# gabrielfnayres/new-vit

Hardware: AMD Instinct MI355X
Metric: volumes_per_sec_mst_dinov2_fwd (higher is better)
Workload: dtype bf16; 1 GPU; MST-DINOv2 (DinoV2ClassifierSlice, ViT-S/14) forward, 4 volumes/GPU of 64x512x512 bf16 zero-padded to 518x518 (N=1370 tokens/slice); global_batch_volumes=4, slices=64, parallelism=single GPU, weights=synthetic (mst.synth seed 2), random init of the reference architecture

## Files before the change

### new-vit_amd/build.py

```python
#!/usr/bin/env python3
from __future__ import annotations

import argparse
import os
import shutil
import subprocess
import sys
from concurrent.futures import ThreadPoolExecutor
from pathlib import Path

HERE = Path(__file__).resolve().parent
CSRC = HERE / "csrc"
OBJ = HERE / "build"
LIB = Path(os.environ.get("MST_BUILD_LIB", HERE / "mst" / "hip" / "libmst_hip.so"))
FLAGS = ["--offload-arch=gfx950", "-O3", "-std=c++17", "-fPIC", "-Wall", "-Wno-unused-function",
         "-Wno-unused-variable", "-Wno-unused-but-set-variable"]
PER_FILE_FLAGS = {"k_block16s.hip": ["-fno-slp-vectorize"],
                  "k_attn16.hip": ["-mllvm", "-amdgpu-mfma-vgpr-form"], "k_attn32.hip": ["-mllvm", "-amdgpu-mfma-vgpr-form"],
                  "k_attn16_train.hip": ["-mllvm", "-amdgpu-mfma-vgpr-form"]}


def hipcc() -> str:
    for c in (os.environ.get("HIPCC"), shutil.which("hipcc"), "/opt/rocm/bin/hipcc"):
        if c and Path(c).exists():
            return c
    raise RuntimeError("hipcc not found (ROCm toolchain required to build libmst_hip.so)")


def newer(src: Path, dst: Path, deps) -> bool:
    if not dst.exists():
        return True
    t = dst.stat().st_mtime
    return any(p.stat().st_mtime > t for p in [src, *deps])


def build(force: bool = False, jobs: int = 8, verbose: bool = True) -> Path:
    global OBJ
    cc = hipcc()
    extra = os.environ.get("MST_EXTRA_FLAGS", "").split()
    if extra:
        OBJ = HERE / ("build_" + "_".join(f.strip("-").replace("=", "") for f in extra))
        FLAGS.extend(f for f in extra if f not in FLAGS)
    OBJ.mkdir(exist_ok=True)
    headers = list(CSRC.glob("*.h")) + [HERE.parent / "include" / "mst_hip.h", Path(__file__)]
    srcs = sorted(CSRC.glob("*.hip"))
    todo = [s for s in srcs if force or newer(s, OBJ / (s.stem + ".o"), headers)]

    def compile_one(src: Path):
        cmd = [cc, *FLAGS, *PER_FILE_FLAGS.get(src.name, []), "-c", str(src), "-o", str(OBJ / (src.stem + ".o"))]
        r = subprocess.run(cmd, capture_output=True, text=True)
        return src, r

    with ThreadPoolExecutor(max_workers=max(1, jobs)) as ex:
        for src, r in ex.map(compile_one, todo):
            if verbose and (r.stderr.strip() or r.returncode):
                sys.stderr.write(r.stderr)
            if r.returncode:
                raise RuntimeError(f"hipcc failed on {src.name}")
            if verbose:
                print(f"[build] {src.name}")
    objs = [OBJ / (s.stem + ".o") for s in srcs]
    if force or todo or not LIB.exists():
        cmd = [cc, "--offload-arch=gfx950", "-shared", "-fPIC", "-o", str(LIB), *map(str, objs)]
        r = subprocess.run(cmd, capture_output=True, text=True)
        if r.returncode:
            sys.stderr.write(r.stderr)
            raise RuntimeError("link failed")
        if verbose:
            print(f"[build] linked {LIB}")
    return LIB


if __name__ == "__main__":
    ap = argparse.ArgumentParser()
    ap.add_argument("--force", action="store_true")
    ap.add_argument("--jobs", type=int, default=8)
    a = ap.parse_args()
    build(a.force, a.jobs)
```

### new-vit_amd/csrc/k_gemm16_wreg.hip

```cpp
#include <cstdlib>

#include "mst_common.h"

namespace {

constexpr int KD = GEMM16_WREG_TILE.bk, BN = GEMM16_WREG_TILE.bn, CH = GEMM16_WREG_TILE.bm;
constexpr int ROWB = KD * 2;
constexpr int SLOT = CH * ROWB;
constexpr int WREG_NSLOT = 4;
constexpr int NSLOT = WREG_NSLOT;
constexpr int STG_PITCH = ROWB + 16;
constexpr int STG_BYTES = CH * STG_PITCH;
constexpr int STG_OFF = NSLOT * SLOT;
constexpr int LDS_BYTES = STG_OFF + 2 * STG_BYTES;
constexpr int NKT = KD / 32;
constexpr int PPW = SLOT / 1024 / 8;
static_assert(NSLOT == 4, "the counted vmcnt table below is written for three chunks in flight");

#define WREG_RD(dst, base, imm) asm volatile("ds_read_b128 %0, %1 offset:%2" : "=v"(dst) : "v"(base), "n"(imm) : "memory")

template <typename T, bool BLK>
__global__ __launch_bounds__(512) __attribute__((amdgpu_waves_per_eu(2, 2))) void gemm16_wreg_kernel(
    const T* __restrict__ A, int64_t lda, const T* __restrict__ W, int64_t ldw, const float* __restrict__ bias, T* __restrict__ C,
    int64_t ldc, int M, int N, float col_scale, int scale_cols, int nchunks) {
    typedef typename V8<T>::type vec8;
    typedef __attribute__((ext_vector_type(4))) T out4;
    extern __shared__ __attribute__((aligned(16))) char smem[];
    const int lane = threadIdx.x & 63;
    const int wave = __builtin_amdgcn_readfirstlane(threadIdx.x >> 6);
    const int frow = lane & 15, kq = lane >> 4;

    const int xcd = blockIdx.x & 7, g = blockIdx.x >> 3, G = gridDim.x >> 3;
    const int tiles_n = N / BN;
    const int nt = g % tiles_n, jcu = g / tiles_n;
    const int c_nt = (G - nt + tiles_n - 1) / tiles_n;
    const int per_xcd = (nchunks + 7) >> 3;
    const int lo = xcd * per_xcd;
    const int hi = lo + per_xcd < nchunks ? lo + per_xcd : nchunks;
    const int n0 = nt * BN + wave * 48;
    const float cs = nt * BN < scale_cols ? col_scale : 1.f;

    vec8 w[3][NKT];
#pragma unroll
    for (int t = 0; t < 3; ++t) {
        const T* wr = W + (int64_t)(n0 + 12 * (frow >> 2) + 4 * t + (frow & 3)) * ldw + kq * 8;
#pragma unroll
        for (int kt = 0; kt < NKT; ++kt) w[t][kt] = *reinterpret_cast<const vec8*>(wr + kt * 32);
    }
    f32x4 b[3];
#pragma unroll
    for (int t = 0; t < 3; ++t) {
        b[t] = (f32x4){0.f, 0.f, 0.f, 0.f};
        if (bias) b[t] = *reinterpret_cast<const f32x4*>(bias + n0 + 12 * kq + 4 * t);
    }
#pragma unroll
    for (int t = 0; t < 3; ++t) {
        asm volatile("" : "+v"(b[t]));
#pragma unroll
        for (int kt = 0; kt < NKT; ++kt) asm volatile("" : "+v"(w[t][kt]));
    }

    unsigned dma_off[PPW];
#pragma unroll
    for (int u = 0; u < PPW; ++u) {
        const int o = (wave * PPW + u) * 1024 + lane * 16;
        const int r = o / ROWB;
        dma_off[u] = BLK ? (unsigned)o : (unsigned)(r * (int)lda * 2 + ((((o % ROWB) >> 4) ^ (r & 15)) << 4));
    }
    const int64_t chunk_bytes = BLK ? (int64_t)SLOT : (int64_t)CH * lda * 2;
    auto issue_piece = [&](int chunk, int slot, int u) {
        const char* base = reinterpret_cast<const char*>(A) + (int64_t)chunk * chunk_bytes;
        unsigned off = dma_off[u];
        const int valid = M - chunk * CH;
        if (!BLK && valid < CH) {
            const int o = (wave * PPW + u) * 1024 + lane * 16;
            int r = o / ROWB;
            const int ck = ((o % ROWB) >> 4) ^ (r & 15);
            r = r < valid ? r : valid - 1;
            off = (unsigned)(r * (int)lda * 2 + ck * 16);
        }
        __builtin_amdgcn_global_load_lds(GLB_PTR(base + off), LDS_PTR(smem + slot * SLOT + (wave * PPW + u) * 1024), 16, 0, 0);
    };

    int rb[4];
#pragma unroll
    for (int j = 0; j < 4; ++j) rb[j] = BLK ? (kq >> 1) * 1024 + (frow + 32 * (kq & 1)) * 16 : frow * ROWB + (((4 * j + kq) ^ frow) << 4);
    const int put_off = frow * STG_PITCH + wave * 96 + kq * 24;
    int fl_lds[3];
    unsigned fl_glb[3];
    int fl_row[3];
#pragma unroll
    for (int j = 0; j < 3; ++j) {
        const int q = lane + 64 * j;
        fl_row[j] = wave * 4 + q / 48;
        fl_lds[j] = fl_row[j] * STG_PITCH + (q % 48) * 16;
        fl_glb[j] = (unsigned)(fl_row[j] * (int)ldc * 2 + nt * BN * 2 + (q % 48) * 16);
    }
    f32x4 acc[2][3];
    auto put = [&](int it) {
        char* stg = smem + STG_OFF + (it & 1) * STG_BYTES + put_off;
#pragma unroll
        for (int mt = 0; mt < 2; ++mt)
#pragma unroll
            for (int t = 0; t < 3; ++t) {
                out4 pk;
#pragma unroll
                for (int i = 0; i < 4; ++i) pk[i] = (T)(acc[mt][t][i] * cs);
                *reinterpret_cast<out4*>(stg + mt * 16 * STG_PITCH + t * 8) = pk;
            }
    };
    auto flush_piece = [&](int chunk, int it, int j) {
        const char* stg = smem + STG_OFF + (it & 1) * STG_BYTES;
        char* cb = reinterpret_cast<char*>(C) + (int64_t)chunk * CH * ldc * 2;
        const int valid = M - chunk * CH;
        const u32x4 v = *reinterpret_cast<const u32x4*>(stg + fl_lds[j]);
        if (valid >= CH || fl_row[j] < valid) {
            __builtin_nontemporal_store(v, reinterpret_cast<u32x4*>(cb + fl_glb[j]));
        }
    };
    auto flush = [&](int chunk, int it) {
#pragma unroll
        for (int j = 0; j < 3; ++j) flush_piece(chunk, it, j);
    };

    int c = lo + jcu;
    if (c >= hi) return;
#pragma unroll
    for (int d = 0; d < NSLOT - 1; ++d)
        if (c + d * c_nt < hi) {
#pragma unroll
            for (int u = 0; u < PPW; ++u) issue_piece(c + d * c_nt, d, u);
        }

    int prev = -1, last_it = 0;
    for (int it = 0; c < hi; c += c_nt, ++it) {
        if (c + 2 * c_nt < hi) {
            if (it <= 1) asm volatile("s_waitcnt vmcnt(6)" ::: "memory");
            else if (it == 2) asm volatile("s_waitcnt vmcnt(9)" ::: "memory");
            else asm volatile("s_waitcnt vmcnt(12)" ::: "memory");
        } else {
            asm volatile("s_waitcnt vmcnt(0)" ::: "memory");
        }
        asm volatile("s_waitcnt lgkmcnt(0)\n\ts_barrier" ::: "memory");
        if (prev >= 0) flush(prev, it - 1);

        const int slot = it % NSLOT;
        const int nxt = c + (NSLOT - 1) * c_nt, nslot = (it + NSLOT - 1) % NSLOT;
        const bool more = nxt < hi;
        int rbs[4];
#pragma unroll
        for (int j = 0; j < 4; ++j) rbs[j] = rb[j] + slot * SLOT;
#pragma unroll
        for (int mt = 0; mt < 2; ++mt)
#pragma unroll
            for (int t = 0; t < 3; ++t) acc[mt][t] = b[t];

        u32x4 a[2][2];
        WREG_RD(a[0][0], rbs[0], 0);
        if constexpr (BLK) WREG_RD(a[0][1], rbs[0], 256);
        else WREG_RD(a[0][1], rbs[0], 16 * ROWB);
#pragma unroll
        for (int kt = 0; kt < NKT; ++kt) {
            const int cur = kt & 1;
            if (kt + 1 < NKT) {
                switch (kt + 1) {
#define WREG_NEXT(KN)                                                                  \
    case KN:                                                                           \
        if constexpr (BLK) {                                                           \
            WREG_RD(a[(KN) & 1][0], rbs[0], (KN) * 2048);                              \
            WREG_RD(a[(KN) & 1][1], rbs[0], (KN) * 2048 + 256);                        \
        } else {                                                                       \
            WREG_RD(a[(KN) & 1][0], rbs[(KN) & 3], ((KN) >> 2) * 256);                 \
            WREG_RD(a[(KN) & 1][1], rbs[(KN) & 3], 16 * ROWB + ((KN) >> 2) * 256);     \
        }                                                                              \
        break;
                    WREG_NEXT(1) WREG_NEXT(2) WREG_NEXT(3) WREG_NEXT(4) WREG_NEXT(5) WREG_NEXT(6)
                    WREG_NEXT(7) WREG_NEXT(8) WREG_NEXT(9) WREG_NEXT(10) WREG_NEXT(11)
#undef WREG_NEXT
                }
                asm volatile("s_waitcnt lgkmcnt(2)" : "+v"(a[cur][0]), "+v"(a[cur][1])::"memory");
            } else {
                asm volatile("s_waitcnt lgkmcnt(0)" : "+v"(a[cur][0]), "+v"(a[cur][1])::"memory");
            }
            const vec8 a0 = __builtin_bit_cast(vec8, a[cur][0]), a1 = __builtin_bit_cast(vec8, a[cur][1]);
#pragma unroll
            for (int t = 0; t < 3; ++t) {
                acc[0][t] = mfma16(w[t][kt], a0, acc[0][t]);
                acc[1][t] = mfma16(w[t][kt], a1, acc[1][t]);
            }
            if ((kt & 3) == 1) {
                __builtin_amdgcn_sched_barrier(0);
                if (more) issue_piece(nxt, nslot, kt >> 2);
                __builtin_amdgcn_sched_barrier(0);
            }
        }
        put(it);
        prev = c;
        last_it = it;
    }
    asm volatile("s_waitcnt lgkmcnt(0)\n\ts_barrier" ::: "memory");
    flush(prev, last_it);
}

template <typename T, bool BLK>
int launch_t(const gemm_args& g) {
    static mst_lds_once lds_once;
    auto kern = gemm16_wreg_kernel<T, BLK>;
    mst_allow_lds((const void*)kern, LDS_BYTES, &lds_once);
    const int nchunks = (int)((g.M + CH - 1) / CH);
    kern<<<dim3(mst_persistent_grid()), dim3(512), LDS_BYTES, g.s>>>((const T*)g.A, g.lda, (const T*)g.W, g.ldw, g.bias, (T*)g.C, g.ldc, (int)g.M,
                                                                      g.N, g.col_scale, g.scale_cols, nchunks);
    return mst_check_launch("gemm16_wreg");
}

}

int launch_gemm16_wreg(const gemm_args& g, int a_blocked) {
    if (a_blocked) {
        if (g.dt == MST_BF16) return launch_t<bf16_t, true>(g);
        if (g.dt == MST_F16) return launch_t<f16_t, true>(g);
    }
    if (g.dt == MST_BF16) return launch_t<bf16_t, false>(g);
    if (g.dt == MST_F16) return launch_t<f16_t, false>(g);
    mst_set_error("gemm16_wreg: bad operand dtype %d", g.dt);
    return MST_EINVAL;
}
```

Measured before the change: 166.3 volumes/s.

## Overlap wreg GEMM output flush with MFMA loop and specialize scaling epilogue

The output-tile flush is split into LDS reads, issued alongside the first A-fragment reads, and buffer stores issued after the first MFMA group. This hides the epilogue store latency behind compute instead of running it serially after the barrier. Row masking now relies on a buffer resource with a bounded extent rather than per-lane branches. The chunk loop is also instantiated separately for scaled and unscaled columns so the multiply is skipped when not needed, with packed conversion (and fma_mix for f16) and -fno-slp-vectorize added for this file. The cost is more live VGPRs for the staged flush data and code duplication from the two loop instantiations.

```diff
diff --git a/new-vit_amd/build.py b/new-vit_amd/build.py
--- a/new-vit_amd/build.py
+++ b/new-vit_amd/build.py
@@ -16,6 +16,7 @@
 FLAGS = ["--offload-arch=gfx950", "-O3", "-std=c++17", "-fPIC", "-Wall", "-Wno-unused-function",
          "-Wno-unused-variable", "-Wno-unused-but-set-variable"]
 PER_FILE_FLAGS = {"k_block16s.hip": ["-fno-slp-vectorize"],
+                  "k_gemm16_wreg.hip": ["-fno-slp-vectorize"],
                   "k_attn16.hip": ["-mllvm", "-amdgpu-mfma-vgpr-form"], "k_attn32.hip": ["-mllvm", "-amdgpu-mfma-vgpr-form"],
                   "k_attn16_train.hip": ["-mllvm", "-amdgpu-mfma-vgpr-form"]}
 
diff --git a/new-vit_amd/csrc/k_gemm16_wreg.hip b/new-vit_amd/csrc/k_gemm16_wreg.hip
--- a/new-vit_amd/csrc/k_gemm16_wreg.hip
+++ b/new-vit_amd/csrc/k_gemm16_wreg.hip
@@ -1,4 +1,5 @@
 #include <cstdlib>
+#include <type_traits>
 
 #include "mst_common.h"
 
@@ -24,7 +25,8 @@
     const T* __restrict__ A, int64_t lda, const T* __restrict__ W, int64_t ldw, const float* __restrict__ bias, T* __restrict__ C,
     int64_t ldc, int M, int N, float col_scale, int scale_cols, int nchunks) {
     typedef typename V8<T>::type vec8;
-    typedef __attribute__((ext_vector_type(4))) T out4;
+    typedef __attribute__((ext_vector_type(2))) T out2;
+    typedef __attribute__((ext_vector_type(2))) float f32x2;
     extern __shared__ __attribute__((aligned(16))) char smem[];
     const int lane = threadIdx.x & 63;
     const int wave = __builtin_amdgcn_readfirstlane(threadIdx.x >> 6);
@@ -38,7 +40,7 @@
     const int lo = xcd * per_xcd;
     const int hi = lo + per_xcd < nchunks ? lo + per_xcd : nchunks;
     const int n0 = nt * BN + wave * 48;
-    const float cs = nt * BN < scale_cols ? col_scale : 1.f;
+    const bool scaled = nt * BN < scale_cols && col_scale != 1.f;
 
     vec8 w[3][NKT];
 #pragma unroll
@@ -88,39 +90,52 @@
     const int put_off = frow * STG_PITCH + wave * 96 + kq * 24;
     int fl_lds[3];
     unsigned fl_glb[3];
-    int fl_row[3];
 #pragma unroll
     for (int j = 0; j < 3; ++j) {
         const int q = lane + 64 * j;
-        fl_row[j] = wave * 4 + q / 48;
-        fl_lds[j] = fl_row[j] * STG_PITCH + (q % 48) * 16;
-        fl_glb[j] = (unsigned)(fl_row[j] * (int)ldc * 2 + nt * BN * 2 + (q % 48) * 16);
+        const int row = wave * 4 + q / 48;
+        fl_lds[j] = row * STG_PITCH + (q % 48) * 16;
+        fl_glb[j] = (unsigned)(row * (int)ldc * 2 + nt * BN * 2 + (q % 48) * 16);
     }
     f32x4 acc[2][3];
-    auto put = [&](int it) {
+    auto put = [&](int it, auto sc_tag) {
+        constexpr bool SC = decltype(sc_tag)::value;
         char* stg = smem + STG_OFF + (it & 1) * STG_BYTES + put_off;
 #pragma unroll
         for (int mt = 0; mt < 2; ++mt)
 #pragma unroll
             for (int t = 0; t < 3; ++t) {
-                out4 pk;
-#pragma unroll
-                for (int i = 0; i < 4; ++i) pk[i] = (T)(acc[mt][t][i] * cs);
-                *reinterpret_cast<out4*>(stg + mt * 16 * STG_PITCH + t * 8) = pk;
+                f32x4 v = acc[mt][t];
+                u32x2 pk;
+                if constexpr (SC && std::is_same<T, f16_t>::value) {
+                    const float m1 = v[1] * col_scale, m2 = v[2] * col_scale;
+                    pk[0] = __builtin_bit_cast(unsigned, __builtin_convertvector((f32x2){m1, m1}, out2));
+                    pk[1] = __builtin_bit_cast(unsigned, __builtin_convertvector((f32x2){m2, m2}, out2));
+                    asm("v_fma_mixlo_f16 %0, %1, %2, 0" : "+v"(pk[0]) : "v"(col_scale), "v"(v[0]));
+                    asm("v_fma_mixhi_f16 %0, %1, %2, 0" : "+v"(pk[1]) : "v"(col_scale), "v"(v[3]));
+                } else {
+                    if constexpr (SC) {
+#pragma unroll
+                        for (int i = 0; i < 4; ++i) v[i] *= col_scale;
+                    }
+                    pk[0] = __builtin_bit_cast(unsigned, __builtin_convertvector((f32x2){v[0], v[1]}, out2));
+                    pk[1] = __builtin_bit_cast(unsigned, __builtin_convertvector((f32x2){v[2], v[3]}, out2));
+                }
+                *reinterpret_cast<u32x2*>(stg + mt * 16 * STG_PITCH + t * 8) = pk;
             }
     };
-    auto flush_piece = [&](int chunk, int it, int j) {
-        const char* stg = smem + STG_OFF + (it & 1) * STG_BYTES;
-        char* cb = reinterpret_cast<char*>(C) + (int64_t)chunk * CH * ldc * 2;
+    u32x4 fl[3] = {};
+    auto flush_reads = [&](int it) {
+        const int tile = STG_OFF + (it & 1) * STG_BYTES;
+#pragma unroll
+        for (int j = 0; j < 3; ++j) WREG_RD(fl[j], fl_lds[j] + tile, 0);
+    };
+    auto flush_stores = [&](int chunk) {
         const int valid = M - chunk * CH;
-        const u32x4 v = *reinterpret_cast<const u32x4*>(stg + fl_lds[j]);
-        if (valid >= CH || fl_row[j] < valid) {
-            __builtin_nontemporal_store(v, reinterpret_cast<u32x4*>(cb + fl_glb[j]));
-        }
-    };
-    auto flush = [&](int chunk, int it) {
-#pragma unroll
-        for (int j = 0; j < 3; ++j) flush_piece(chunk, it, j);
+        const __amdgpu_buffer_rsrc_t rows = __builtin_amdgcn_make_buffer_rsrc(
+            reinterpret_cast<char*>(C) + (int64_t)chunk * CH * ldc * 2, 0, (valid < CH ? valid : CH) * (int)ldc * 2, 0x00020000);
+#pragma unroll
+        for (int j = 0; j < 3; ++j) __builtin_amdgcn_raw_buffer_store_b128(fl[j], rows, (int)fl_glb[j], 0, 2);
     };
 
     int c = lo + jcu;
@@ -133,37 +148,38 @@
         }
 
     int prev = -1, last_it = 0;
-    for (int it = 0; c < hi; c += c_nt, ++it) {
-        if (c + 2 * c_nt < hi) {
-            if (it <= 1) asm volatile("s_waitcnt vmcnt(6)" ::: "memory");
-            else if (it == 2) asm volatile("s_waitcnt vmcnt(9)" ::: "memory");
-            else asm volatile("s_waitcnt vmcnt(12)" ::: "memory");
-        } else {
-            asm volatile("s_waitcnt vmcnt(0)" ::: "memory");
-        }
-        asm volatile("s_waitcnt lgkmcnt(0)\n\ts_barrier" ::: "memory");
-        if (prev >= 0) flush(prev, it - 1);
-
-        const int slot = it % NSLOT;
-        const int nxt = c + (NSLOT - 1) * c_nt, nslot = (it + NSLOT - 1) % NSLOT;
-        const bool more = nxt < hi;
-        int rbs[4];
-#pragma unroll
-        for (int j = 0; j < 4; ++j) rbs[j] = rb[j] + slot * SLOT;
-#pragma unroll
-        for (int mt = 0; mt < 2; ++mt)
-#pragma unroll
-            for (int t = 0; t < 3; ++t) acc[mt][t] = b[t];
-
-        u32x4 a[2][2];
-        WREG_RD(a[0][0], rbs[0], 0);
-        if constexpr (BLK) WREG_RD(a[0][1], rbs[0], 256);
-        else WREG_RD(a[0][1], rbs[0], 16 * ROWB);
-#pragma unroll
-        for (int kt = 0; kt < NKT; ++kt) {
-            const int cur = kt & 1;
-            if (kt + 1 < NKT) {
-                switch (kt + 1) {
+    auto chunks = [&](auto sc_tag) {
+        for (int it = 0; c < hi; c += c_nt, ++it) {
+            if (c + 2 * c_nt < hi) {
+                if (it <= 1) asm volatile("s_waitcnt vmcnt(6)" ::: "memory");
+                else if (it == 2) asm volatile("s_waitcnt vmcnt(9)" ::: "memory");
+                else asm volatile("s_waitcnt vmcnt(12)" ::: "memory");
+            } else {
+                asm volatile("s_waitcnt vmcnt(0)" ::: "memory");
+            }
+            asm volatile("s_waitcnt lgkmcnt(0)\n\ts_barrier" ::: "memory");
+
+            const int slot = it % NSLOT;
+            const int nxt = c + (NSLOT - 1) * c_nt, nslot = (it + NSLOT - 1) % NSLOT;
+            const bool more = nxt < hi;
+            int rbs[4];
+#pragma unroll
+            for (int j = 0; j < 4; ++j) rbs[j] = rb[j] + slot * SLOT;
+#pragma unroll
+            for (int mt = 0; mt < 2; ++mt)
+#pragma unroll
+                for (int t = 0; t < 3; ++t) acc[mt][t] = b[t];
+
+            u32x4 a[2][2];
+            WREG_RD(a[0][0], rbs[0], 0);
+            if constexpr (BLK) WREG_RD(a[0][1], rbs[0], 256);
+            else WREG_RD(a[0][1], rbs[0], 16 * ROWB);
+            if (prev >= 0) flush_reads(it - 1);
+#pragma unroll
+            for (int kt = 0; kt < NKT; ++kt) {
+                const int cur = kt & 1;
+                if (kt + 1 < NKT) {
+                    switch (kt + 1) {
 #define WREG_NEXT(KN)                                                                  \
     case KN:                                                                           \
         if constexpr (BLK) {                                                           \
@@ -174,32 +190,43 @@
             WREG_RD(a[(KN) & 1][1], rbs[(KN) & 3], 16 * ROWB + ((KN) >> 2) * 256);     \
         }                                                                              \
         break;
-                    WREG_NEXT(1) WREG_NEXT(2) WREG_NEXT(3) WREG_NEXT(4) WREG_NEXT(5) WREG_NEXT(6)
-                    WREG_NEXT(7) WREG_NEXT(8) WREG_NEXT(9) WREG_NEXT(10) WREG_NEXT(11)
+                        WREG_NEXT(1) WREG_NEXT(2) WREG_NEXT(3) WREG_NEXT(4) WREG_NEXT(5) WREG_NEXT(6)
+                        WREG_NEXT(7) WREG_NEXT(8) WREG_NEXT(9) WREG_NEXT(10) WREG_NEXT(11)
 #undef WREG_NEXT
-                }
-                asm volatile("s_waitcnt lgkmcnt(2)" : "+v"(a[cur][0]), "+v"(a[cur][1])::"memory");
-            } else {
-                asm volatile("s_waitcnt lgkmcnt(0)" : "+v"(a[cur][0]), "+v"(a[cur][1])::"memory");
+                    }
+                    if (kt == 0) asm volatile("s_waitcnt lgkmcnt(2)" : "+v"(a[0][0]), "+v"(a[0][1]), "+v"(fl[0]), "+v"(fl[1]), "+v"(fl[2])::"memory");
+                    else asm volatile("s_waitcnt lgkmcnt(2)" : "+v"(a[cur][0]), "+v"(a[cur][1])::"memory");
+                } else {
+                    asm volatile("s_waitcnt lgkmcnt(0)" : "+v"(a[cur][0]), "+v"(a[cur][1])::"memory");
+                }
+                const vec8 a0 = __builtin_bit_cast(vec8, a[cur][0]), a1 = __builtin_bit_cast(vec8, a[cur][1]);
+#pragma unroll
+                for (int t = 0; t < 3; ++t) {
+                    acc[0][t] = mfma16(w[t][kt], a0, acc[0][t]);
+                    acc[1][t] = mfma16(w[t][kt], a1, acc[1][t]);
+                }
+                if (kt == 0 && prev >= 0) {
+                    __builtin_amdgcn_sched_barrier(0);
+                    flush_stores(prev);
+                    __builtin_amdgcn_sched_barrier(0);
+                }
+                if ((kt & 3) == 1) {
+                    __builtin_amdgcn_sched_barrier(0);
+                    if (more) issue_piece(nxt, nslot, kt >> 2);
+                    __builtin_amdgcn_sched_barrier(0);
+                }
             }
-            const vec8 a0 = __builtin_bit_cast(vec8, a[cur][0]), a1 = __builtin_bit_cast(vec8, a[cur][1]);
-#pragma unroll
-            for (int t = 0; t < 3; ++t) {
-                acc[0][t] = mfma16(w[t][kt], a0, acc[0][t]);
-                acc[1][t] = mfma16(w[t][kt], a1, acc[1][t]);
-            }
-            if ((kt & 3) == 1) {
-                __builtin_amdgcn_sched_barrier(0);
-                if (more) issue_piece(nxt, nslot, kt >> 2);
-                __builtin_amdgcn_sched_barrier(0);
-            }
+            put(it, sc_tag);
+            prev = c;
+            last_it = it;
         }
-        put(it);
-        prev = c;
-        last_it = it;
-    }
+    };
+    if (scaled) chunks(std::true_type{});
+    else chunks(std::false_type{});
     asm volatile("s_waitcnt lgkmcnt(0)\n\ts_barrier" ::: "memory");
-    flush(prev, last_it);
+    flush_reads(last_it);
+    asm volatile("s_waitcnt lgkmcnt(0)" : "+v"(fl[0]), "+v"(fl[1]), "+v"(fl[2])::"memory");
+    flush_stores(prev);
 }
 
 template <typename T, bool BLK>
```

New measurement: 167.8 volumes/s, median of 6. Within noise of the previous version (+0.9%).
